# kawshik8/GAN-Image-Captioning

Measured on NVIDIA B200. Metric: adversarial_train_steps_per_sec, higher is better.
Workload: dtype bf16 operands on the discriminator's highway/dx/dW_h contractions, tf32 on the others (fp32 accumulate)

## Files before the change

gan-image-captioning_b200/_lib.py:

```python
from __future__ import annotations

import ctypes as C
import os
import re

HERE = os.path.dirname(os.path.abspath(__file__))
LIB_PATH = os.path.join(HERE, "libgic_b200.so")
HEADER = os.path.join(os.path.dirname(HERE), "include", "gic_b200.h")

GEMM_FP32, GEMM_TF32, GEMM_BF16 = 0, 1, 3
LOSS_TYPES = {"standard": 0, "JS": 1, "KL": 2, "hinge": 3, "tv": 4, "rsgan": 5}

_lib = None


class AttnBlock(C.Structure):
    _fields_ = [("grid", C.c_void_p), ("P", C.c_int), ("Cf", C.c_int), ("Da", C.c_int), ("W_k", C.c_void_p),
                ("W_v", C.c_void_p), ("W_q", C.c_void_p), ("w_e", C.c_void_p), ("saved", C.c_void_p), ("ws", C.c_void_p),
                ("dW_k", C.c_void_p), ("dW_v", C.c_void_p), ("dW_q", C.c_void_p), ("dw_e", C.c_void_p)]


def attn_block(grid, W_k, W_v, W_q, w_e, saved, ws=None, dW_k=None, dW_v=None, dW_q=None, dw_e=None):
    B, Pn, Cf = grid.shape
    return AttnBlock(ptr(grid), Pn, Cf, W_k.shape[0], ptr(W_k), ptr(W_v), ptr(W_q), ptr(w_e), ptr(saved), ptr(ws),
# ... 47 lines not shown
    L.gic_encoder_bwd.argtypes = [I, P, P, P, P, P, P, P, I, I, I, P, P, P, P, P, I, P]
    L.gic_encoder_bn_running_update.argtypes = [P, P, I, F, F, F, P, P, P, P]
    L.gic_encoder_fwd_eval.argtypes = [I, P, I, I, I, P, P, P, P, F, P, P, P, P, P]
    L.gic_sample_step.argtypes = [I, P, P, F, I, I, I, I, P, P, P, P, I, P, P]
    for f in (L.gic_decode_saved_floats, L.gic_decode_fwd_workspace_floats, L.gic_decode_bwd_workspace_floats,
              L.gic_disc_saved_floats, L.gic_disc_fwd_workspace_floats, L.gic_disc_bwd_workspace_floats,
              L.gic_disc_bwd_demb_offset_floats):
        f.restype = Z
    L.gic_decode_saved_floats.argtypes = [I] * 5
    L.gic_decode_fwd_workspace_floats.argtypes = [I] * 3
    L.gic_decode_bwd_workspace_floats.argtypes = [I] * 6
    L.gic_disc_saved_floats.argtypes = [I] * 5
    L.gic_disc_fwd_workspace_floats.argtypes = [I]
    L.gic_disc_bwd_workspace_floats.argtypes = [I] * 5
    L.gic_disc_bwd_demb_offset_floats.argtypes = [I] * 5
    L.gic_decode_sample_bwd_factored.argtypes = [I, P, P, P, I, P, P, P, P, P, P, F, I, I, I, I, I, I, P, P, P, P, P, P,
                                                 P, P, P, P, I, P]
    L.gic_decode_sample_fwd.argtypes = [I, P, P, P, P, P, P, P, P, P, F, I, P, I, I, I, I, I, I, P, P, P, P, P]
    L.gic_decode_sample_bwd.argtypes = [I, P, P, P, P, P, P, P, F, I, I, I, I, I, I, I, P, P, P, P, P, P, P, P, P, P,
                                        I, P]
    L.gic_disc_fwd.argtypes = [I, P, P, I, I, I, I, I, I, P, P, P, P, P, P, P, P, P, I, P, P, I, P, F, P, P, P, P]
    L.gic_disc_bwd.argtypes = [I, P, P, F, P, P, I, I, I, I, I, I, P, P, P, P, P, P, P, P, I, P, P, P, P, P, P, P, P,
                               P, P, P, P, P, P, I, I, P]
    L.gic_gan_loss_fwd_bwd.argtypes = [I, P, P, P, I, P, P, P, P, P]
    L.gic_grad_sqnorm.argtypes = [P, Z, P, P]
    L.gic_clip_adam.argtypes = [P, P, P, P, Z, P, F, F, I, F, F, F, F, P]
    L.gic_clip_adam_dyn.argtypes = [P, P, P, P, Z, P, F, F, P, F, F, F, P]
    L.gic_decode_sample_cdf_fwd.argtypes = [I, P, P, P, P, P, P, P, P, P, P, I, I, I, I, I, I, P, P, P, P, P, P]
    L.gic_attn_saved_floats.restype = Z
    L.gic_attn_saved_floats.argtypes = [I] * 5
    L.gic_attn_bwd_workspace_floats.restype = Z
    L.gic_attn_bwd_workspace_floats.argtypes = [I] * 5
    L.gic_decode_sample_fwd_attn.argtypes = [P] + [I, P, P, P, P, P, P, P, P, P, F, I, P, I, I, I, I, I, I, P, P, P, P, P]
    L.gic_decode_sample_bwd_attn.argtypes = [P, I, P, P, P, P, I, P, P, P, P, P, P, F, I, I, I, I, I, I, I, P, P, P, P, P,
                                             P, P, P, P, P, P]
    L.gic_sample_cdf_step.argtypes = [P, P, I, I, I, I, P, P, P, P, P, I, P, P]
    L.gic_decode_rollouts_workspace_floats.restype = Z
    L.gic_decode_rollouts_workspace_floats.argtypes = [I] * 6
    L.gic_decode_rollouts.argtypes = [I, P, P, P, P, P, P, P, P, P, P, I, I, I, I, I, I, P, P, P]
    L.gic_rollout_rewards.argtypes = [P, P, I, I, I, I, P, P]
    L.gic_ce_loss_fwd_bwd.argtypes = [P, P, I, I, I, P, P, P]
    L.gic_pg_loss_fwd_bwd.argtypes = [P, P, P, I, I, I, I, P, P, P, P]
    L.gic_set_temperature_device.restype = None
    L.gic_set_temperature_device.argtypes = [P]
    L.gic_disc_prepared_floats.restype = Z
    L.gic_disc_prepared_floats.argtypes = [I]
# ... 199 lines not shown
```

gan-image-captioning_b200/csrc/capi.cu:

```cuda
#include "../../include/gic_b200.h"
#include <stdlib.h>
#include <new>

#include "gic_internal.cuh"

namespace gic {
int gather_rows(const float*, const int64_t*, int, int, int, float*, cudaStream_t);
int vec_add(const float*, const float*, int, float*, cudaStream_t);
int sample_step(bool, const float*, const float*, float, int, int, int, int, float*, int64_t*, const int64_t*,
                const float*, int, float*, cudaStream_t, bool fast_math = false);
int softmax_bwd(const float*, const float*, float, int, int, float*, cudaStream_t);
int rowdot(const float*, const float*, int, int, float*, cudaStream_t);
int sample_cdf_step(const float*, const float*, int, int, int, int, long long, float*, int64_t*, float*, const int64_t*,
                    const float*, int, float*, cudaStream_t);
int rollout_init(const float*, const float*, const int64_t*, const float*, int, int, int, int, int, int, int, float*,
                 float*, float*, int64_t*, cudaStream_t);
int softmax_bwd_dot(const float*, const float*, const float*, float, int, int, float*, cudaStream_t);
int softmax_bwd_dot_bf16(const float*, const float*, const float*, float, int, int, void*, int, cudaStream_t);
int colsum_bf16(const void*, int, int, int, bool, float*, cudaStream_t);
int embed_scatter(const float*, const int64_t*, int, int, int, int, float*, float*, cudaStream_t);
int bn_fwd(const float*, int, int, const float*, const float*, float, float*, float*, float*, cudaStream_t);
int bn_bwd(const float*, const float*, int, int, const float*, const float*, const float*, float*, float*, float*,
           cudaStream_t);
int lstm_cell_fwd(const float*, const float*, int, int, float*, float*, float*, float*, int, int, cudaStream_t);
// ... 52 lines not shown
int pack_captions(const int32_t*, const int32_t*, int, int, int64_t*, int32_t*, cudaStream_t);
const float* temperature_device();
void disc_set_prepared(const float*);
int disc_prepare(int, const float*, const float*, const float*, int, const float*, const float*, int, float*, cudaStream_t);
size_t disc_fwd_workspace_floats(int);
const char* last_error();
unsigned long long launch_count();
unsigned long long kernel_launches(const char*);
int kernel_names(char*, int);
void prof_begin();
void prof_end(double*, double*, unsigned long long*);
int disc_fwd_entry(int mode, const float* inp_soft, const int64_t* ids, int N, int L, int V, int De, int R,
                   int n_groups, const int* fs, const int* nf, const float* W_e, const float* const* cw,
                   const float* const* cb, const float* W_h, const float* b_h, const float* W_f, const float* b_f,
                   int Hd, const float* W_o, const float* b_o, int n_heads, const uint8_t* const* keep, float drop_p,
                   float* const* logits, float* saved, float* ws, cudaStream_t s);
int disc_bwd_entry(int mode, const float* dlogits, const uint8_t* keep, float drop_p, const float* inp_soft,
                   const int64_t* ids, int N, int L, int V, int De, int R, int n_groups, const int* fs, const int* nf,
                   const float* W_e, const float* const* cw, const float* const* cb, const float* W_h,
                   const float* W_f, const float* b_f, int Hd, const float* W_o, const float* b_o, const float* saved,
                   float* ws, float* dW_e, float* const* dcw, float* const* dcb, float* dW_h, float* db_h,
                   float* dW_f, float* db_f, float* dW_o, float* db_o, float* dinp, int want_param, int accumulate,
                   cudaStream_t s);

static size_t a4(size_t x) { return (x + 3) & ~(size_t)3; }

struct AttnLayout {
  size_t Ak, Av, q, alpha, total;
  size_t dAk, dAv, dq, ds, ws_total;
  AttnLayout(int B, int L, int P, int Da, int E) {
    Ak = 0; Av = a4((size_t)B * P * Da); q = Av + a4((size_t)B * P * E); alpha = q + a4((size_t)L * B * Da);
    total = alpha + a4((size_t)L * B * P);
    dAk = 0; dAv = a4((size_t)B * P * Da); dq = dAv + a4((size_t)B * P * E); ds = dq + a4((size_t)L * B * Da);
    ws_total = ds + a4((size_t)L * B * P);
  }
};

struct DecodeSaved {
  size_t xs, hs0, cs0, acts0, per_layer, htop, total;
  DecodeSaved(int B, int L, int E, int H, int layers) {
    const size_t BH = (size_t)B * H;
    xs = 0;
    size_t off = a4((size_t)L * B * E);
    hs0 = off;
    cs0 = hs0 + a4((size_t)(L + 1) * BH);
    acts0 = cs0 + a4((size_t)(L + 1) * BH);
// ... 703 lines not shown
                 int n_groups, const int* filter_sizes, const int* num_filters, const float* W_e,
                 const float* const* conv_w, const float* const* conv_b, const float* W_h, const float* b_h,
                 const float* W_f, const float* b_f, int Hd, const float* W_o, const float* b_o, int n_heads,
                 const uint8_t* const* keep, float drop_p, float* const* logits, float* saved, float* workspace,
                 gic_stream_t stream) {
  GIC_TRY(require_device());
  return disc_fwd_entry(mode, inp_soft, ids, N, L, V, De, R, n_groups, filter_sizes, num_filters, W_e, conv_w, conv_b,
                        W_h, b_h, W_f, b_f, Hd, W_o, b_o, n_heads, keep, drop_p, logits, saved, workspace, S(stream));
}

int gic_disc_bwd(int mode, const float* dlogits, const uint8_t* keep, float drop_p, const float* inp_soft,
                 const int64_t* ids, int N, int L, int V, int De, int R, int n_groups, const int* filter_sizes,
                 const int* num_filters, const float* W_e, const float* const* conv_w, const float* const* conv_b,
                 const float* W_h, const float* W_f, const float* b_f, int Hd, const float* W_o, const float* b_o,
                 const float* saved, float* workspace, float* dW_e, float* const* dconv_w, float* const* dconv_b,
                 float* dW_h, float* db_h, float* dW_f, float* db_f, float* dW_o, float* db_o, float* dinp,
                 int want_param, int accumulate, gic_stream_t stream) {
  GIC_TRY(require_device());
  return disc_bwd_entry(mode, dlogits, keep, drop_p, inp_soft, ids, N, L, V, De, R, n_groups, filter_sizes,
                        num_filters, W_e, conv_w, conv_b, W_h, W_f, b_f, Hd, W_o, b_o, saved, workspace, dW_e, dconv_w,
                        dconv_b, dW_h, db_h, dW_f, db_f, dW_o, db_o, dinp, want_param, accumulate, S(stream));
}

int gic_gan_loss_fwd_bwd(int loss_type, const float* d_out_real, const float* d_out_fake, const float* g_out, int n,
                         float* losses, float* dd_real, float* dd_fake, float* dg_out, gic_stream_t stream) {
  GIC_TRY(require_device());
  return gan_loss(loss_type, d_out_real, d_out_fake, g_out, n, losses, dd_real, dd_fake, dg_out, S(stream));
}

int gic_grad_sqnorm(const float* g, size_t n, float* sqnorm, gic_stream_t stream) {
  GIC_TRY(require_device());
  return grad_sqnorm(g, n, sqnorm, S(stream));
}

int gic_clip_adam(float* p, const float* g, float* m, float* v, size_t n, const float* sqnorm, float max_norm,
                  float grad_scale, int step, float lr, float beta1, float beta2, float eps, gic_stream_t stream) {
  GIC_TRY(require_device());
  return clip_adam(p, g, m, v, n, sqnorm, max_norm, grad_scale, step, lr, beta1, beta2, eps, nullptr, S(stream));
}

int gic_clip_adam_dyn(float* p, const float* g, float* m, float* v, size_t n, const float* sqnorm, float max_norm,
                      float grad_scale, const float* bias_corr_dev, float beta1, float beta2, float eps,
                      gic_stream_t stream) {
  GIC_TRY(require_device());
  GIC_REQUIRE(bias_corr_dev, GIC_ERR_NULL, "clip_adam_dyn: NULL bias_corr_dev");
  return clip_adam(p, g, m, v, n, sqnorm, max_norm, grad_scale, 0, 0.f, beta1, beta2, eps, bias_corr_dev, S(stream));
// ... 59 lines not shown
```

gan-image-captioning_b200/csrc/disc.cu:

```cuda
#include <stdlib.h>

#include "gic_internal.cuh"

namespace gic {

constexpr int MAX_GROUPS = 8;

__device__ __forceinline__ unsigned long long pack2(float lo, float hi) {
  unsigned long long r;
  asm("mov.b64 %0, {%1, %2};" : "=l"(r) : "f"(lo), "f"(hi));
  return r;
}
__device__ __forceinline__ void unpack2(unsigned long long v, float& lo, float& hi) {
  asm("mov.b64 {%0, %1}, %2;" : "=f"(lo), "=f"(hi) : "l"(v));
}
__device__ __forceinline__ unsigned long long ffma2(unsigned long long a, unsigned long long b, unsigned long long c) {
  unsigned long long d;
  asm("fma.rn.f32x2 %0, %1, %2, %3;" : "=l"(d) : "l"(a), "l"(b), "l"(c));
  return d;
}

__device__ __forceinline__ unsigned short f2bf(float x) {
  unsigned int u = __float_as_uint(x);
  u += 0x7fffu + ((u >> 16) & 1u);
// ... 462 lines not shown
      const int row = rb + j;
      const bool ok = active && row < r1;
      const size_t i = (size_t)row * F + c;
      gv[j] = ok ? dx[i] + dx2[i] : 0.f;
      av[j] = ok ? (int)arg[i] : ARG_DEAD;
    }
    __syncthreads();
#pragma unroll
    for (int j = 0; j < DW_RC; ++j) {
      if (av[j] != ARG_DEAD && gv[j] != 0.f) {
        const float* e0 = sm + j * LE + av[j] * es;
#pragma unroll
        for (int k = 0; k < BWD_KMAX; ++k)
          if (k < fk) dw[k] = fmaf(gv[j], e0[k], dw[k]);
        dbias += gv[j];
      }
    }
  }
  if (!active) return;
#pragma unroll
  for (int k = 0; k < BWD_KMAX; ++k)
    if (k < fk) atomicAdd(g.dw[gi] + cin * fk + k, dw[k]);
  atomicAdd(g.db[gi] + cin, dbias);
}

__global__ void __launch_bounds__(256)
head_collapse_kernel(const float* __restrict__ W_f, const float* __restrict__ b_f,
                     const float* __restrict__ w_o, const float* __restrict__ b_o, int F,
                     int Hd, float* __restrict__ weff ) {
  __shared__ float part[8][33];
  const int lane = threadIdx.x & 31, w = threadIdx.x >> 5;
  const int j = blockIdx.x * 32 + lane;
  float s = 0.f;
  if (j < F) {
#pragma unroll 4
    for (int k = w; k < Hd; k += 8) s = fmaf(w_o[k], W_f[(size_t)k * F + j], s);
  } else if (j == F) {
    for (int k = w; k < Hd; k += 8) s = fmaf(w_o[k], b_f[k], s);
  }
  part[w][lane] = s;
  __syncthreads();
  if (w == 0 && j <= F) {
    float t = (j == F) ? b_o[0] : 0.f;
#pragma unroll
    for (int i = 0; i < 8; ++i) t += part[i][lane];
    weff[j] = t;
// ... 256 lines not shown
static size_t align4(size_t x) { return (x + 3) & ~(size_t)3; }

static inline int bf_pitch(int F) { return ((F + 63) / 64) * 64; }

size_t disc_saved_floats(int N, int L, int De, int R, int F) {
  const size_t rows = (size_t)N * R;
  return align4((size_t)N * L * De) + 2 * align4(rows * F) + align4((rows * F + 3) / 4) + align4(rows * bf_pitch(F) / 2);
}
size_t disc_fwd_workspace_floats(int F) { return align4((size_t)F + 1) + align4((size_t)F * bf_pitch(F) / 2); }
size_t disc_bwd_workspace_floats(int N, int L, int De, int R, int F) {
  const size_t rows = (size_t)N * R;
  const size_t dh = align4(rows * F) > align4(rows * bf_pitch(F) / 2) ? align4(rows * F) : align4(rows * bf_pitch(F) / 2);
  return align4((size_t)F + 1) + dh + align4(rows * F) + 2 * align4(F) + align4((size_t)N * L * De) +
         align4((size_t)F * bf_pitch(F) / 2) + align4(rows * F);
}

int disc_fill_groups(ConvGroups& g, int ngroups, const int* fs, const int* nf, const float* const* cw,
                     const float* const* cb, float* const* dcw, float* const* dcb, int es) {
  GIC_REQUIRE(ngroups >= 1 && ngroups <= MAX_GROUPS, GIC_ERR_SHAPE, "disc: 1..%d filter groups supported", MAX_GROUPS);
  g.ngroups = ngroups; g.F = 0; g.kmax = 0;
  for (int i = 0; i < MAX_GROUPS; ++i) { g.w[i] = g.b[i] = nullptr; g.dw[i] = g.db[i] = nullptr; g.f[i] = g.n[i] = g.col0[i] = 0; }
  for (int i = 0; i < ngroups; ++i) {
    GIC_REQUIRE(fs[i] >= 1 && nf[i] >= 1, GIC_ERR_SHAPE, "disc: bad filter group %d", i);
    GIC_REQUIRE(cw[i] && cb[i], GIC_ERR_NULL, "disc: NULL conv weights for group %d", i);
    g.w[i] = cw[i]; g.b[i] = cb[i];
    g.dw[i] = dcw ? dcw[i] : nullptr; g.db[i] = dcb ? dcb[i] : nullptr;
    g.f[i] = fs[i]; g.n[i] = nf[i]; g.col0[i] = g.F; g.F += nf[i];
    if (fs[i] * es > g.kmax) g.kmax = fs[i] * es;
  }
  return GIC_OK;
}

void disc_set_prepared(const float* prep) { ctx().prepared = prep; }
#define g_prepared (ctx().prepared)

int disc_prepare(int mode, const float* W_h, const float* W_f, const float* b_f, int Hd, const float* W_o,
                 const float* b_o, int F, float* prep, cudaStream_t s) {
  GIC_REQUIRE(W_h && W_f && b_f && W_o && b_o && prep, GIC_ERR_NULL, "disc_prepare: NULL pointer");
  GIC_REQUIRE(F >= 1 && Hd >= 1, GIC_ERR_SHAPE, "disc_prepare: bad shape");
  head_collapse_kernel<<<cdiv(F + 1, 32), 256, 0, s>>>(W_f, b_f, W_o, b_o, F, Hd, prep);
  GIC_TRY(check_launch("head_collapse_kernel"));
  if (mode == GEMM_BF16 && (F % 4 == 0)) {
    unsigned short* W_h_bf = reinterpret_cast<unsigned short*>(prep + align4((size_t)F + 1));
    GIC_TRY(f32_to_bf16(W_h, F, F, F, W_h_bf, bf_pitch(F), s));
  }
  return GIC_OK;
}

// ... 78 lines not shown
  }
  HeadPtrs hp;
  hp.n = n_heads;
  for (int m = 0; m < MAX_HEADS; ++m) {
    hp.keep[m] = (m < n_heads && keep) ? keep[m] : nullptr;
    hp.logits[m] = (m < n_heads) ? logits[m] : nullptr;
  }
  ProfScope prof(PROF_HEAD, (8.0 + n_heads) * rows * d.F, s);
  bool vec = (d.F % 4 == 0) && d.F <= 4 * 32 * 8;
  for (int m = 0; m < n_heads; ++m) vec = vec && (!hp.keep[m] || (reinterpret_cast<uintptr_t>(hp.keep[m]) & 3u) == 0);
  if (vec) {
    const int nq = cdiv(d.F / 4, 32);
    const int grid = cdiv((long long)rows, 8);
    const float dsc = 1.f / (1.f - drop_p);
    const bool fast = (mode == GEMM_TF32 || mode == GEMM_BF16);
#define GIC_HF(NQ_) do { if (fast) head_fwd_vec_kernel<NQ_, true><<<grid, 256, 0, s>>>(hpre, pooled, (int)rows, d.F, weff, dsc, hp); \
                         else head_fwd_vec_kernel<NQ_, false><<<grid, 256, 0, s>>>(hpre, pooled, (int)rows, d.F, weff, dsc, hp); } while (0)
    if (nq <= 2) GIC_HF(2); else if (nq <= 4) GIC_HF(4); else GIC_HF(8);
#undef GIC_HF
  } else {
    head_fwd_kernel<<<cdiv((long long)rows, 8), 256, 0, s>>>(hpre, pooled, (int)rows, d.F, weff, 1.f / (1.f - drop_p), hp);
  }
  return check_launch("head_fwd_kernel");
}

int disc_backward(int mode, const float* dlogit, const uint8_t* keep, float drop_p, const float* inp_soft,
                  const int64_t* ids, const DiscDims& d, ConvGroups& g, const float* W_e, const float* W_h,
                  const float* W_f, const float* b_f, const float* W_o, const float* b_o, const float* saved,
                  float* ws, float* dW_e, float* dW_h, float* db_h, float* dW_f, float* db_f, float* dW_o,
                  float* db_o, float* dinp, int want_param, int accumulate, cudaStream_t s) {
  const size_t rows = d.rows();
  if (d.N == 0) return GIC_OK;
  const float* emb = saved;
  const float* pooled = emb + align4((size_t)d.N * d.L * d.De);
  const float* hpre = pooled + align4(rows * d.F);
  const uint8_t* arg = reinterpret_cast<const uint8_t*>(hpre + align4(rows * d.F));
  const bool bf = (mode == GEMM_BF16) && (d.F % 4 == 0) && (!keep || (reinterpret_cast<uintptr_t>(keep) & 3u) == 0);
  const int Fp = bf_pitch(d.F);
  const unsigned short* pooled_bf =
      reinterpret_cast<const unsigned short*>(reinterpret_cast<const float*>(arg) + align4((rows * d.F + 3) / 4));
  const float* prep = g_prepared;
  const float* weff = prep ? prep : ws;
  float* dh = ws + align4((size_t)d.F + 1);
  const size_t dh_floats = align4(rows * d.F) > align4(rows * Fp / 2) ? align4(rows * d.F) : align4(rows * Fp / 2);
  float* dx = dh + dh_floats;
  float* sacc = dx + align4(rows * d.F);
// ... 28 lines not shown
    const int colb = cdiv(d.F, 256);
    int chunks = max(1, (4 * num_sms()) / colb);
    int rpc = cdiv((long long)rows, chunks);
    chunks = cdiv((long long)rows, rpc);
    head_bwd_kernel<<<dim3(colb, chunks), 256, 0, s>>>(dlogit, keep, 1.f / (1.f - drop_p), hpre, pooled, (int)rows,
                                                      d.F, weff, rpc, dh, dx, sacc, dbh);
    GIC_TRY(check_launch("head_bwd_kernel"));
  }
  if (want_param) {
    head_param_grads_kernel<<<d.Hd, 256, 0, s>>>(dlogit, (int)rows, sacc, dbh, W_f, b_f, W_o, d.F, d.Hd, beta, dW_f,
                                                db_f, dW_o, db_o, db_h);
    GIC_TRY(check_launch("head_param_grads_kernel"));
    if (bf)
      GIC_TRY(gemm_bf16(true, false, d.F, d.F, (int)rows, 1.f, dh, Fp, pooled_bf, Fp, beta, dW_h, d.F, nullptr, s, PROF_GEMM_D));
    else
      GIC_TRY(gemm(mode, true, false, d.F, d.F, (int)rows, 1.f, dh, d.F, pooled, d.F, beta, dW_h, d.F, nullptr, s, PROF_GEMM_D));
  }
  if (bf) {
    if (!prep) GIC_TRY(f32_to_bf16(W_h, d.F, d.F, d.F, W_h_bf_ws, Fp, s));
    GIC_TRY(gemm_bf16(false, false, (int)rows, d.F, d.F, 1.f, dh, Fp, W_h_bf, Fp, 0.f, dxg, d.F, nullptr, s, PROF_GEMM_D));
  } else {
    GIC_TRY(gemm(mode, false, false, (int)rows, d.F, d.F, 1.f, dh, d.F, W_h, d.F, 0.f, dxg, d.F, nullptr, s, PROF_GEMM_D));
  }
  {
    GIC_REQUIRE(g.kmax <= BWD_KMAX, GIC_ERR_SHAPE, "disc bwd: filter_size*emb_dim_single <= %d supported", BWD_KMAX);
    if (want_param && !accumulate) {
      for (int i = 0; i < g.ngroups; ++i) {
        cudaMemsetAsync(g.dw[i], 0, (size_t)g.n[i] * g.f[i] * d.es * sizeof(float), s);
        cudaMemsetAsync(g.db[i], 0, (size_t)g.n[i] * sizeof(float), s);
      }
    }
    {
      const size_t fixed = ((size_t)g.kmax + 1) * d.F * 4;
      const size_t per_warp = (size_t)d.L * d.es * 32 * 4;
      int nwarps = 8;
      while (nwarps > 1 && fixed + nwarps * per_warp > 100 * 1024) nwarps >>= 1;
      const size_t smem = fixed + nwarps * per_warp;
      GIC_REQUIRE(smem <= 200 * 1024, GIC_ERR_SHAPE, "disc bwd: L*emb_dim_single too large for shared memory");
      const int grid = min(cdiv((long long)rows, nwarps), 4 * num_sms());
      bool vec = (d.F % 4 == 0) && aligned16(dx) && aligned16(dxg) && ((reinterpret_cast<uintptr_t>(arg) & 3u) == 0);
      for (int i = 0; i < g.ngroups; ++i) vec = vec && (g.n[i] % 4 == 0);
      static bool attr = false;
      if (!attr) {
        cudaFuncSetAttribute(conv_pool_bwd_demb_kernel<true, true>, cudaFuncAttributeMaxDynamicSharedMemorySize, 200 * 1024);
        cudaFuncSetAttribute(conv_pool_bwd_demb_kernel<true, false>, cudaFuncAttributeMaxDynamicSharedMemorySize, 200 * 1024);
        cudaFuncSetAttribute(conv_pool_bwd_demb_kernel<false, true>, cudaFuncAttributeMaxDynamicSharedMemorySize, 200 * 1024);
        cudaFuncSetAttribute(conv_pool_bwd_demb_kernel<false, false>, cudaFuncAttributeMaxDynamicSharedMemorySize, 200 * 1024);
        attr = true;
      }
#define GIC_DEMB(ES1_, VEC_) conv_pool_bwd_demb_kernel<ES1_, VEC_><<<grid, nwarps * 32, smem, s>>>(arg, dx, dxg, (int)rows, d.L, d.De, d.R, d.es, g, demb)
      if (d.es == 1) { if (vec) GIC_DEMB(true, true); else GIC_DEMB(true, false); }
      else { if (vec) GIC_DEMB(false, true); else GIC_DEMB(false, false); }
#undef GIC_DEMB
      GIC_TRY(check_launch("conv_pool_bwd_demb_kernel"));
    }
    if (want_param) {
      const int colb = cdiv(d.F, 256);
      int per_sm = 4;
      { const int o = option("GIC_DW_CTAS_PER_SM", 0); if (o > 0) per_sm = o; }
      int chunks = max(1, (per_sm * num_sms()) / colb);
      int rpc = cdiv((long long)rows, chunks);
      rpc = ((rpc + DW_RC - 1) / DW_RC) * DW_RC;
      chunks = cdiv((long long)rows, rpc);
      const size_t smem = (size_t)DW_RC * d.L * d.es * 4;
      GIC_REQUIRE(smem <= 48 * 1024, GIC_ERR_SHAPE, "disc bwd: L*emb_dim_single too large for shared memory");
      if (d.es == 1)
        conv_pool_bwd_dw_kernel<true><<<dim3(colb, chunks), 256, smem, s>>>(emb, arg, dx, dxg, (int)rows, d.L, d.De, d.R, d.es, g, rpc);
      else
        conv_pool_bwd_dw_kernel<false><<<dim3(colb, chunks), 256, smem, s>>>(emb, arg, dx, dxg, (int)rows, d.L, d.De, d.R, d.es, g, rpc);
      GIC_TRY(check_launch("conv_pool_bwd_dw_kernel"));
    }
  }
  if (want_param) {
    if (inp_soft) {
      GIC_TRY(gemm(mode, true, false, d.De, d.V, d.N * d.L, 1.f, demb, d.De, inp_soft, d.V, beta, dW_e, d.V, nullptr, s));
    } else {
      if (!accumulate) cudaMemsetAsync(dW_e, 0, (size_t)d.De * d.V * sizeof(float), s);
      const int tot = d.N * d.L * d.De;
      disc_embed_ids_bwd_kernel<<<cdiv(tot, 256), 256, 0, s>>>(ids, d.N * d.L, d.V, d.De, demb, dW_e);
      GIC_TRY(check_launch("disc_embed_ids_bwd_kernel"));
    }
  }
  if (dinp) {
    GIC_TRY(gemm(mode, false, false, d.N * d.L, d.V, d.De, 1.f, demb, d.De, W_e, d.V, 0.f, dinp, d.V, nullptr, s));
  }
  return GIC_OK;
}

static int disc_dims(DiscDims& d, int N, int L, int V, int De, int R, int Hd, const ConvGroups& g) {
  GIC_REQUIRE(N >= 0 && L >= 1 && V >= 1 && De >= 1 && R >= 1 && Hd >= 1, GIC_ERR_SHAPE, "disc: bad shape");
  GIC_REQUIRE(De % R == 0, GIC_ERR_SHAPE, "disc: disc_embed_dim %d not divisible by disc_num_rep %d", De, R);
  d.N = N; d.L = L; d.V = V; d.De = De; d.R = R; d.es = De / R; d.F = g.F; d.Hd = Hd; d.ngroups = g.ngroups;
  d.kmax = g.kmax;
  for (int i = 0; i < g.ngroups; ++i)
    GIC_REQUIRE(L >= g.f[i], GIC_ERR_SHAPE, "disc: caption length %d shorter than filter size %d", L, g.f[i]);
// ... 23 lines not shown

int disc_bwd_entry(int mode, const float* dlogits, const uint8_t* keep, float drop_p, const float* inp_soft,
                   const int64_t* ids, int N, int L, int V, int De, int R, int n_groups, const int* fs, const int* nf,
                   const float* W_e, const float* const* cw, const float* const* cb, const float* W_h,
                   const float* W_f, const float* b_f, int Hd, const float* W_o, const float* b_o, const float* saved,
                   float* ws, float* dW_e, float* const* dcw, float* const* dcb, float* dW_h, float* db_h,
                   float* dW_f, float* db_f, float* dW_o, float* db_o, float* dinp, int want_param, int accumulate,
                   cudaStream_t s) {
  GIC_REQUIRE((inp_soft != nullptr) != (ids != nullptr), GIC_ERR_NULL, "disc_bwd: exactly one of inp_soft / ids");
  GIC_REQUIRE(dlogits && fs && nf && cw && cb && W_e && W_h && W_f && b_f && W_o && b_o && saved && ws, GIC_ERR_NULL,
              "disc_bwd: NULL pointer");
  GIC_REQUIRE(!want_param || (dW_e && dcw && dcb && dW_h && db_h && dW_f && db_f && dW_o && db_o), GIC_ERR_NULL,
              "disc_bwd: NULL gradient buffer");
  GIC_REQUIRE(!(dinp && ids), GIC_ERR_UNSUPPORTED, "disc_bwd: hard-token input has no gradient");
  const int es = (R > 0 && De % R == 0) ? De / R : 1;
  ConvGroups g;
  GIC_TRY(disc_fill_groups(g, n_groups, fs, nf, cw, cb, want_param ? dcw : nullptr, want_param ? dcb : nullptr, es));
  DiscDims d;
  GIC_TRY(disc_dims(d, N, L, V, De, R, Hd, g));
  return disc_backward(mode, dlogits, keep, drop_p, inp_soft, ids, d, g, W_e, W_h, W_f, b_f, W_o, b_o, saved, ws, dW_e,
                       dW_h, db_h, dW_f, db_f, dW_o, db_o, dinp, want_param, accumulate, s);
}

}
```

include/gic_b200.h:

```cpp
#ifndef GIC_B200_H_
#define GIC_B200_H_

#include <stddef.h>
#include <stdint.h>

#ifdef __cplusplus
extern "C" {
#endif

typedef void* gic_stream_t;

#define GIC_OK 0
#define GIC_ERR_SHAPE 1
#define GIC_ERR_NULL 2
#define GIC_ERR_CUDA 3
#define GIC_ERR_WORKSPACE 4
#define GIC_ERR_ARCH 5
#define GIC_ERR_UNSUPPORTED 6

#define GIC_GEMM_FP32 0
#define GIC_GEMM_TF32 1
#define GIC_GEMM_BF16 3

#define GIC_LOSS_STANDARD 0
// ... 64 lines not shown
                                   float temperature, int B, int L, int V, int E, int H, int layers, const float* saved,
                                   float* workspace, float* dW_emb, float* const* dW_ih, float* const* dW_hh,
                                   float* const* db_ih, float* const* db_hh, float* dW_out, float* db_out,
                                   float* dfeatures, int accumulate, gic_stream_t stream);

size_t gic_disc_saved_floats(int N, int L, int De, int R, int F);
size_t gic_disc_fwd_workspace_floats(int F);
int gic_disc_fwd(int mode, const float* inp_soft, const int64_t* ids, int N, int L, int V, int De, int R,
                 int n_groups, const int* filter_sizes, const int* num_filters, const float* W_e ,
                 const float* const* conv_w, const float* const* conv_b, const float* W_h ,
                 const float* b_h, const float* W_f , const float* b_f, int Hd, const float* W_o ,
                 const float* b_o, int n_heads, const uint8_t* const* keep, float drop_p, float* const* logits,
                 float* saved, float* workspace, gic_stream_t stream);

size_t gic_disc_bwd_workspace_floats(int N, int L, int De, int R, int F);
size_t gic_disc_bwd_demb_offset_floats(int N, int L, int De, int R, int F);
int gic_disc_bwd(int mode, const float* dlogits, const uint8_t* keep, float drop_p, const float* inp_soft,
                 const int64_t* ids, int N, int L, int V, int De, int R, int n_groups, const int* filter_sizes,
                 const int* num_filters, const float* W_e, const float* const* conv_w, const float* const* conv_b,
                 const float* W_h, const float* W_f, const float* b_f, int Hd, const float* W_o, const float* b_o,
                 const float* saved, float* workspace, float* dW_e, float* const* dconv_w, float* const* dconv_b,
                 float* dW_h, float* db_h, float* dW_f, float* db_f, float* dW_o, float* db_o, float* dinp,
                 int want_param, int accumulate, gic_stream_t stream);

int gic_gan_loss_fwd_bwd(int loss_type, const float* d_out_real, const float* d_out_fake, const float* g_out, int n,
                         float* losses, float* dd_real, float* dd_fake, float* dg_out, gic_stream_t stream);

int gic_grad_sqnorm(const float* g, size_t n, float* sqnorm, gic_stream_t stream);
int gic_clip_adam(float* p, const float* g, float* m, float* v, size_t n, const float* sqnorm, float max_norm,
                  float grad_scale, int step, float lr, float beta1, float beta2, float eps, gic_stream_t stream);

int gic_ce_loss_fwd_bwd(const float* logits , const int64_t* targets , int B, int L, int V,
                        float* loss , float* dlogits , gic_stream_t stream);

int gic_sample_cdf_step(const float* logits, const float* u, int B, int V, int L, int t, float* out, int64_t* ids,
                        float* logp, const int64_t* forced_ids, const float* embed, int E, float* x_next,
                        gic_stream_t stream);
int gic_decode_sample_cdf_fwd(int mode, const float* features, const float* W_emb, const float* const* W_ih,
                              const float* const* W_hh, const float* const* b_ih, const float* const* b_hh,
                              const float* W_out, const float* b_out, const float* u, const int64_t* forced_ids, int B,
                              int L, int V, int E, int H, int layers, float* logits_out, int64_t* ids, float* logp,
                              float* saved, float* workspace, gic_stream_t stream);
size_t gic_decode_rollouts_workspace_floats(int B, int L, int V, int E, int H, int n_roll);
int gic_decode_rollouts(int mode, const float* saved, const int64_t* main_ids, const float* W_emb, const float* W_ih,
                        const float* W_hh, const float* b_ih, const float* b_hh, const float* W_out,
                        const float* b_out, const float* u_roll, int B, int L, int V, int E, int H, int n_roll,
// ... 110 lines not shown
```

Measured before the change: 459.3.

## Fuse conv-pool backward demb and weight-gradient passes into one kernel

```diff
diff --git a/gan-image-captioning_b200/_lib.py b/gan-image-captioning_b200/_lib.py
--- a/gan-image-captioning_b200/_lib.py
+++ b/gan-image-captioning_b200/_lib.py
@@ -93,6 +93,7 @@
     L.gic_disc_fwd.argtypes = [I, P, P, I, I, I, I, I, I, P, P, P, P, P, P, P, P, P, I, P, P, I, P, F, P, P, P, P]
     L.gic_disc_bwd.argtypes = [I, P, P, F, P, P, I, I, I, I, I, I, P, P, P, P, P, P, P, P, I, P, P, P, P, P, P, P, P,
                                P, P, P, P, P, P, I, I, P]
+    L.gic_conv_pool_bwd.argtypes = [P, P, P, P, I, I, I, I, I, P, P, P, P, P, P, I, I, P]
     L.gic_gan_loss_fwd_bwd.argtypes = [I, P, P, P, I, P, P, P, P, P]
     L.gic_grad_sqnorm.argtypes = [P, Z, P, P]
     L.gic_clip_adam.argtypes = [P, P, P, P, Z, P, F, F, I, F, F, F, F, P]
diff --git a/gan-image-captioning_b200/csrc/capi.cu b/gan-image-captioning_b200/csrc/capi.cu
--- a/gan-image-captioning_b200/csrc/capi.cu
+++ b/gan-image-captioning_b200/csrc/capi.cu
@@ -98,6 +98,9 @@
                    float* ws, float* dW_e, float* const* dcw, float* const* dcb, float* dW_h, float* db_h,
                    float* dW_f, float* db_f, float* dW_o, float* db_o, float* dinp, int want_param, int accumulate,
                    cudaStream_t s);
+int conv_pool_bwd_entry(const uint8_t* arg, const float* dx, const float* dx2, const float* emb, int N, int L, int De, int R,
+                        int n_groups, const int* fs, const int* nf, const float* const* cw, float* const* dcw,
+                        float* const* dcb, float* demb, int want_param, int accumulate, cudaStream_t s);
 
 static size_t a4(size_t x) { return (x + 3) & ~(size_t)3; }
 
@@ -847,6 +850,15 @@
                         dconv_b, dW_h, db_h, dW_f, db_f, dW_o, db_o, dinp, want_param, accumulate, S(stream));
 }
 
+int gic_conv_pool_bwd(const uint8_t* arg, const float* dx, const float* dx2, const float* emb, int N, int L, int De, int R,
+                      int n_groups, const int* filter_sizes, const int* num_filters, const float* const* conv_w,
+                      float* const* dconv_w, float* const* dconv_b, float* demb, int want_param, int accumulate,
+                      gic_stream_t stream) {
+  GIC_TRY(require_device());
+  return conv_pool_bwd_entry(arg, dx, dx2, emb, N, L, De, R, n_groups, filter_sizes, num_filters, conv_w, dconv_w, dconv_b,
+                             demb, want_param, accumulate, S(stream));
+}
+
 int gic_gan_loss_fwd_bwd(int loss_type, const float* d_out_real, const float* d_out_fake, const float* g_out, int n,
                          float* losses, float* dd_real, float* dd_fake, float* dg_out, gic_stream_t stream) {
   GIC_TRY(require_device());
diff --git a/gan-image-captioning_b200/csrc/disc.cu b/gan-image-captioning_b200/csrc/disc.cu
--- a/gan-image-captioning_b200/csrc/disc.cu
+++ b/gan-image-captioning_b200/csrc/disc.cu
@@ -508,6 +508,164 @@
   for (int k = 0; k < BWD_KMAX; ++k)
     if (k < fk) atomicAdd(g.dw[gi] + cin * fk + k, dw[k]);
   atomicAdd(g.db[gi] + cin, dbias);
+}
+
+template <bool WANT_PARAM, int QPL, int KM>
+__global__ void __launch_bounds__(256, QPL * (KM + 1) <= 12 ? 2 : 1)
+conv_pool_bwd_fused_kernel(const float* __restrict__ emb, const uint8_t* __restrict__ arg, const float* __restrict__ dx,
+                           const float* __restrict__ dx2, int rows, int L, int R, ConvGroups g, int qs,
+                           int rows_per_cta, float* __restrict__ demb, int demb_atomic) {
+  extern __shared__ __align__(16) float sm[];
+  const int F = g.F, F4 = F >> 2;
+  const int nwarps = blockDim.x >> 5, warp = threadIdx.x >> 5, lane = threadIdx.x & 31;
+  const int q_lo = blockIdx.x * qs, nq = min(qs, F4 - q_lo);
+  float4* wk_s = reinterpret_cast<float4*>(sm);
+  float4* red_s = wk_s + (size_t)KM * qs;
+  float* priv = reinterpret_cast<float*>(red_s + (WANT_PARAM ? (size_t)(KM + 1) * qs : 0)) + (size_t)warp * 33 * 32;
+  float* erow = priv + 32 * 32;
+  for (int i = threadIdx.x; i < KM * nq; i += blockDim.x) {
+    const int k = i / nq, ql = i % nq, c = 4 * (q_lo + ql);
+    int gi = 0;
+    while (gi + 1 < g.ngroups && c >= g.col0[gi + 1]) ++gi;
+    const int f = g.f[gi];
+    const float* w = g.w[gi] + (size_t)(c - g.col0[gi]) * f + k;
+    wk_s[k * qs + ql] = (k < f) ? make_float4(w[0], w[f], w[2 * f], w[3 * f]) : make_float4(0.f, 0.f, 0.f, 0.f);
+  }
+  if (WANT_PARAM)
+    for (int i = threadIdx.x; i < (KM + 1) * qs; i += blockDim.x) red_s[i] = make_float4(0.f, 0.f, 0.f, 0.f);
+  int fk[QPL];
+#pragma unroll
+  for (int j = 0; j < QPL; ++j) {
+    const int ql = 32 * j + lane;
+    fk[j] = 0;
+    if (ql < nq) {
+      const int c = 4 * (q_lo + ql);
+      int gi = 0;
+      while (gi + 1 < g.ngroups && c >= g.col0[gi + 1]) ++gi;
+      fk[j] = g.f[gi];
+    }
+  }
+  float4 dw[QPL][KM + 1];
+  if (WANT_PARAM) {
+#pragma unroll
+    for (int j = 0; j < QPL; ++j)
+#pragma unroll
+      for (int k = 0; k <= KM; ++k) dw[j][k] = make_float4(0.f, 0.f, 0.f, 0.f);
+  }
+  __syncthreads();
+
+  const int r0 = blockIdx.y * rows_per_cta, r1 = min(rows, r0 + rows_per_cta);
+  float4 gv[QPL], hv[QPL];
+  uint32_t av[QPL];
+  float ev = 0.f;
+  auto load = [&](int row) {
+    const size_t base = (size_t)row * F;
+    const float4* dx4 = reinterpret_cast<const float4*>(dx + base) + q_lo;
+    const float4* dy4 = reinterpret_cast<const float4*>(dx2 + base) + q_lo;
+    const uint32_t* a4 = reinterpret_cast<const uint32_t*>(arg + base) + q_lo;
+    const bool live = row < r1;
+#pragma unroll
+    for (int j = 0; j < QPL; ++j) {
+      const int ql = 32 * j + lane;
+      const bool ok = live && ql < nq;
+      gv[j] = ok ? dx4[ql] : make_float4(0.f, 0.f, 0.f, 0.f);
+      hv[j] = ok ? dy4[ql] : make_float4(0.f, 0.f, 0.f, 0.f);
+      av[j] = ok ? __ldg(a4 + ql) : 0xffffffffu;
+    }
+    if (WANT_PARAM) ev = (live && lane < L) ? emb[((size_t)(row / R) * L + lane) * R + row % R] : 0.f;
+  };
+  int row = r0 + warp;
+  load(row);
+  for (; row < r1; row += nwarps) {
+    float4 gc[QPL];
+    uint32_t ac[QPL];
+#pragma unroll
+    for (int j = 0; j < QPL; ++j) {
+      gc[j] = make_float4(gv[j].x + hv[j].x, gv[j].y + hv[j].y, gv[j].z + hv[j].z, gv[j].w + hv[j].w);
+      ac[j] = av[j];
+    }
+    if (WANT_PARAM) erow[lane] = ev;
+    load(row + nwarps);
+    for (int t = 0; t < L; ++t) priv[t * 32 + lane] = 0.f;
+    __syncwarp();
+#pragma unroll
+    for (int j = 0; j < QPL; ++j) {
+      const float gg[4] = {gc[j].x, gc[j].y, gc[j].z, gc[j].w};
+      const int aa[4] = {(int)(ac[j] & 0xffu), (int)((ac[j] >> 8) & 0xffu), (int)((ac[j] >> 16) & 0xffu), (int)(ac[j] >> 24)};
+      bool on[4];
+      bool any = false;
+#pragma unroll
+      for (int e = 0; e < 4; ++e) { on[e] = (aa[e] != ARG_DEAD) && (gg[e] != 0.f); any |= on[e]; }
+      if (!any) continue;
+      const int f = fk[j];
+      float4 w4[KM];
+#pragma unroll
+      for (int k = 0; k < KM; ++k) if (k < f) w4[k] = wk_s[k * qs + 32 * j + lane];
+#pragma unroll
+      for (int e = 0; e < 4; ++e) {
+        if (!on[e]) continue;
+        float* p = priv + aa[e] * 32 + lane;
+        const float* er = erow + aa[e];
+#pragma unroll
+        for (int k = 0; k < KM; ++k) {
+          if (k < f) {
+            const float wk = e == 0 ? w4[k].x : e == 1 ? w4[k].y : e == 2 ? w4[k].z : w4[k].w;
+            p[k * 32] = fmaf(wk, gg[e], p[k * 32]);
+            if (WANT_PARAM) {
+              float& d = e == 0 ? dw[j][k].x : e == 1 ? dw[j][k].y : e == 2 ? dw[j][k].z : dw[j][k].w;
+              d = fmaf(gg[e], er[k], d);
+            }
+          }
+        }
+        if (WANT_PARAM) {
+          float& d = e == 0 ? dw[j][KM].x : e == 1 ? dw[j][KM].y : e == 2 ? dw[j][KM].z : dw[j][KM].w;
+          d += gg[e];
+        }
+      }
+    }
+    __syncwarp();
+    if (lane < L) {
+      float acc = 0.f;
+#pragma unroll 8
+      for (int i = 0; i < 32; ++i) acc += priv[lane * 32 + ((i + lane) & 31)];
+      float* o = demb + ((size_t)(row / R) * L + lane) * R + row % R;
+      if (!demb_atomic) *o = acc;
+      else if (acc != 0.f) atomicAdd(o, acc);
+    }
+    __syncwarp();
+  }
+  if (!WANT_PARAM) return;
+  for (int w = 0; w < nwarps; ++w) {
+    if (warp == w) {
+#pragma unroll
+      for (int j = 0; j < QPL; ++j) {
+        const int ql = 32 * j + lane;
+        if (ql >= nq) continue;
+#pragma unroll
+        for (int k = 0; k <= KM; ++k) {
+          float4 v = red_s[k * qs + ql];
+          v.x += dw[j][k].x; v.y += dw[j][k].y; v.z += dw[j][k].z; v.w += dw[j][k].w;
+          red_s[k * qs + ql] = v;
+        }
+      }
+    }
+    __syncthreads();
+  }
+  for (int i = threadIdx.x; i < (KM + 1) * nq; i += blockDim.x) {
+    const int k = i / nq, ql = i % nq, c = 4 * (q_lo + ql);
+    int gi = 0;
+    while (gi + 1 < g.ngroups && c >= g.col0[gi + 1]) ++gi;
+    const int f = g.f[gi], cin = c - g.col0[gi];
+    const float4 v = red_s[k * qs + ql];
+    const float vv[4] = {v.x, v.y, v.z, v.w};
+    if (k == KM) {
+#pragma unroll
+      for (int e = 0; e < 4; ++e) atomicAdd(g.db[gi] + cin + e, vv[e]);
+    } else if (k < f) {
+#pragma unroll
+      for (int e = 0; e < 4; ++e) atomicAdd(g.dw[gi] + (size_t)(cin + e) * f + k, vv[e]);
+    }
+  }
 }
 
 __global__ void __launch_bounds__(256)
@@ -810,8 +968,8 @@
   for (int i = 0; i < MAX_GROUPS; ++i) { g.w[i] = g.b[i] = nullptr; g.dw[i] = g.db[i] = nullptr; g.f[i] = g.n[i] = g.col0[i] = 0; }
   for (int i = 0; i < ngroups; ++i) {
     GIC_REQUIRE(fs[i] >= 1 && nf[i] >= 1, GIC_ERR_SHAPE, "disc: bad filter group %d", i);
-    GIC_REQUIRE(cw[i] && cb[i], GIC_ERR_NULL, "disc: NULL conv weights for group %d", i);
-    g.w[i] = cw[i]; g.b[i] = cb[i];
+    GIC_REQUIRE(cw[i] && (!cb || cb[i]), GIC_ERR_NULL, "disc: NULL conv weights for group %d", i);
+    g.w[i] = cw[i]; g.b[i] = cb ? cb[i] : nullptr;
     g.dw[i] = dcw ? dcw[i] : nullptr; g.db[i] = dcb ? dcb[i] : nullptr;
     g.f[i] = fs[i]; g.n[i] = nf[i]; g.col0[i] = g.F; g.F += nf[i];
     if (fs[i] * es > g.kmax) g.kmax = fs[i] * es;
@@ -936,6 +1094,100 @@
     head_fwd_kernel<<<cdiv((long long)rows, 8), 256, 0, s>>>(hpre, pooled, (int)rows, d.F, weff, 1.f / (1.f - drop_p), hp);
   }
   return check_launch("head_fwd_kernel");
+}
+
+int conv_pool_bwd(const uint8_t* arg, const float* dx, const float* dx2, const float* emb, int N, int L, int De, int R,
+                  const ConvGroups& g, float* demb, int want_param, int accumulate, cudaStream_t s) {
+  const int es = De / R;
+  const size_t rows = (size_t)N * R;
+  GIC_REQUIRE(g.kmax <= BWD_KMAX, GIC_ERR_SHAPE, "disc bwd: filter_size*emb_dim_single <= %d supported", BWD_KMAX);
+  if (want_param && !accumulate) {
+    for (int i = 0; i < g.ngroups; ++i) {
+      cudaMemsetAsync(g.dw[i], 0, (size_t)g.n[i] * g.f[i] * es * sizeof(float), s);
+      cudaMemsetAsync(g.db[i], 0, (size_t)g.n[i] * sizeof(float), s);
+    }
+  }
+  if (rows == 0) return GIC_OK;
+  bool vec = (g.F % 4 == 0) && aligned16(dx) && aligned16(dx2) && ((reinterpret_cast<uintptr_t>(arg) & 3u) == 0);
+  for (int i = 0; i < g.ngroups; ++i) vec = vec && (g.n[i] % 4 == 0);
+  if (vec && es == 1 && L <= 32 && option("GIC_CONV_BWD_FUSED", 1) != 0) {
+    const int km = g.kmax <= 5 ? 5 : 8;
+    int qpl = km == 5 ? 4 : 2;
+    if (km == 5 && option("GIC_CONV_BWD_QPL", 0) == 2) qpl = 2;
+    const int F4 = g.F / 4;
+    const int slices = cdiv(F4, 32 * qpl), qs = cdiv(F4, slices);
+    const size_t smem = (size_t)km * qs * 16 + (want_param ? (size_t)(km + 1) * qs * 16 : 0) + (size_t)8 * 33 * 32 * 4;
+    static bool attr = false;
+    if (!attr) {
+#define GIC_FATTR(P_, Q_, K_) cudaFuncSetAttribute(conv_pool_bwd_fused_kernel<P_, Q_, K_>, cudaFuncAttributeMaxDynamicSharedMemorySize, 200 * 1024)
+      GIC_FATTR(true, 4, 5); GIC_FATTR(true, 2, 5); GIC_FATTR(true, 2, 8);
+      GIC_FATTR(false, 4, 5); GIC_FATTR(false, 2, 5); GIC_FATTR(false, 2, 8);
+#undef GIC_FATTR
+      attr = true;
+    }
+#define GIC_FUSED(P_, Q_, K_)                                                                                               \
+    do {                                                                                                                    \
+      static size_t occ_smem = 0;                                                                                           \
+      static int occ = 1;                                                                                                   \
+      if (occ_smem != smem) {                                                                                               \
+        cudaOccupancyMaxActiveBlocksPerMultiprocessor(&occ, conv_pool_bwd_fused_kernel<P_, Q_, K_>, 256, smem);           \
+        occ = max(occ, 1);                                                                                                  \
+        occ_smem = smem;                                                                                                    \
+      }                                                                                                                     \
+      int chunks = max(1, (occ * num_sms()) / slices);                                                                      \
+      const int rpc = (int)cdiv((long long)rows, chunks);                                                                   \
+      chunks = (int)cdiv((long long)rows, rpc);                                                                             \
+      conv_pool_bwd_fused_kernel<P_, Q_, K_><<<dim3(slices, chunks), 256, smem, s>>>(emb, arg, dx, dx2, (int)rows, L, R,   \
+                                                                                      g, qs, rpc, demb, slices > 1);       \
+    } while (0)
+    if (slices > 1) cudaMemsetAsync(demb, 0, (size_t)N * L * De * sizeof(float), s);
+    if (want_param) {
+      if (km == 8) GIC_FUSED(true, 2, 8); else if (qpl == 2) GIC_FUSED(true, 2, 5); else GIC_FUSED(true, 4, 5);
+    } else {
+      if (km == 8) GIC_FUSED(false, 2, 8); else if (qpl == 2) GIC_FUSED(false, 2, 5); else GIC_FUSED(false, 4, 5);
+    }
+#undef GIC_FUSED
+    return check_launch("conv_pool_bwd_fused_kernel");
+  }
+  {
+    const size_t fixed = ((size_t)g.kmax + 1) * g.F * 4;
+    const size_t per_warp = (size_t)L * es * 32 * 4;
+    int nwarps = 8;
+    while (nwarps > 1 && fixed + nwarps * per_warp > 100 * 1024) nwarps >>= 1;
+    const size_t smem = fixed + nwarps * per_warp;
+    GIC_REQUIRE(smem <= 200 * 1024, GIC_ERR_SHAPE, "disc bwd: L*emb_dim_single too large for shared memory");
+    const int grid = min(cdiv((long long)rows, nwarps), 4 * num_sms());
+    static bool attr = false;
+    if (!attr) {
+      cudaFuncSetAttribute(conv_pool_bwd_demb_kernel<true, true>, cudaFuncAttributeMaxDynamicSharedMemorySize, 200 * 1024);
+      cudaFuncSetAttribute(conv_pool_bwd_demb_kernel<true, false>, cudaFuncAttributeMaxDynamicSharedMemorySize, 200 * 1024);
+      cudaFuncSetAttribute(conv_pool_bwd_demb_kernel<false, true>, cudaFuncAttributeMaxDynamicSharedMemorySize, 200 * 1024);
+      cudaFuncSetAttribute(conv_pool_bwd_demb_kernel<false, false>, cudaFuncAttributeMaxDynamicSharedMemorySize, 200 * 1024);
+      attr = true;
+    }
+#define GIC_DEMB(ES1_, VEC_) conv_pool_bwd_demb_kernel<ES1_, VEC_><<<grid, nwarps * 32, smem, s>>>(arg, dx, dx2, (int)rows, L, De, R, es, g, demb)
+    if (es == 1) { if (vec) GIC_DEMB(true, true); else GIC_DEMB(true, false); }
+    else { if (vec) GIC_DEMB(false, true); else GIC_DEMB(false, false); }
+#undef GIC_DEMB
+    GIC_TRY(check_launch("conv_pool_bwd_demb_kernel"));
+  }
+  if (want_param) {
+    const int colb = cdiv(g.F, 256);
+    int per_sm = 4;
+    { const int o = option("GIC_DW_CTAS_PER_SM", 0); if (o > 0) per_sm = o; }
+    int chunks = max(1, (per_sm * num_sms()) / colb);
+    int rpc = cdiv((long long)rows, chunks);
+    rpc = ((rpc + DW_RC - 1) / DW_RC) * DW_RC;
+    chunks = cdiv((long long)rows, rpc);
+    const size_t smem = (size_t)DW_RC * L * es * 4;
+    GIC_REQUIRE(smem <= 48 * 1024, GIC_ERR_SHAPE, "disc bwd: L*emb_dim_single too large for shared memory");
+    if (es == 1)
+      conv_pool_bwd_dw_kernel<true><<<dim3(colb, chunks), 256, smem, s>>>(emb, arg, dx, dx2, (int)rows, L, De, R, es, g, rpc);
+    else
+      conv_pool_bwd_dw_kernel<false><<<dim3(colb, chunks), 256, smem, s>>>(emb, arg, dx, dx2, (int)rows, L, De, R, es, g, rpc);
+    GIC_TRY(check_launch("conv_pool_bwd_dw_kernel"));
+  }
+  return GIC_OK;
 }
 
 int disc_backward(int mode, const float* dlogit, const uint8_t* keep, float drop_p, const float* inp_soft,
@@ -1010,55 +1262,7 @@
   } else {
     GIC_TRY(gemm(mode, false, false, (int)rows, d.F, d.F, 1.f, dh, d.F, W_h, d.F, 0.f, dxg, d.F, nullptr, s, PROF_GEMM_D));
   }
-  {
-    GIC_REQUIRE(g.kmax <= BWD_KMAX, GIC_ERR_SHAPE, "disc bwd: filter_size*emb_dim_single <= %d supported", BWD_KMAX);
-    if (want_param && !accumulate) {
-      for (int i = 0; i < g.ngroups; ++i) {
-        cudaMemsetAsync(g.dw[i], 0, (size_t)g.n[i] * g.f[i] * d.es * sizeof(float), s);
-        cudaMemsetAsync(g.db[i], 0, (size_t)g.n[i] * sizeof(float), s);
-      }
-    }
-    {
-      const size_t fixed = ((size_t)g.kmax + 1) * d.F * 4;
-      const size_t per_warp = (size_t)d.L * d.es * 32 * 4;
-      int nwarps = 8;
-      while (nwarps > 1 && fixed + nwarps * per_warp > 100 * 1024) nwarps >>= 1;
-      const size_t smem = fixed + nwarps * per_warp;
-      GIC_REQUIRE(smem <= 200 * 1024, GIC_ERR_SHAPE, "disc bwd: L*emb_dim_single too large for shared memory");
-      const int grid = min(cdiv((long long)rows, nwarps), 4 * num_sms());
-      bool vec = (d.F % 4 == 0) && aligned16(dx) && aligned16(dxg) && ((reinterpret_cast<uintptr_t>(arg) & 3u) == 0);
-      for (int i = 0; i < g.ngroups; ++i) vec = vec && (g.n[i] % 4 == 0);
-      static bool attr = false;
-      if (!attr) {
-        cudaFuncSetAttribute(conv_pool_bwd_demb_kernel<true, true>, cudaFuncAttributeMaxDynamicSharedMemorySize, 200 * 1024);
-        cudaFuncSetAttribute(conv_pool_bwd_demb_kernel<true, false>, cudaFuncAttributeMaxDynamicSharedMemorySize, 200 * 1024);
-        cudaFuncSetAttribute(conv_pool_bwd_demb_kernel<false, true>, cudaFuncAttributeMaxDynamicSharedMemorySize, 200 * 1024);
-        cudaFuncSetAttribute(conv_pool_bwd_demb_kernel<false, false>, cudaFuncAttributeMaxDynamicSharedMemorySize, 200 * 1024);
-        attr = true;
-      }
-#define GIC_DEMB(ES1_, VEC_) conv_pool_bwd_demb_kernel<ES1_, VEC_><<<grid, nwarps * 32, smem, s>>>(arg, dx, dxg, (int)rows, d.L, d.De, d.R, d.es, g, demb)
-      if (d.es == 1) { if (vec) GIC_DEMB(true, true); else GIC_DEMB(true, false); }
-      else { if (vec) GIC_DEMB(false, true); else GIC_DEMB(false, false); }
-#undef GIC_DEMB
-      GIC_TRY(check_launch("conv_pool_bwd_demb_kernel"));
-    }
-    if (want_param) {
-      const int colb = cdiv(d.F, 256);
-      int per_sm = 4;
-      { const int o = option("GIC_DW_CTAS_PER_SM", 0); if (o > 0) per_sm = o; }
-      int chunks = max(1, (per_sm * num_sms()) / colb);
-      int rpc = cdiv((long long)rows, chunks);
-      rpc = ((rpc + DW_RC - 1) / DW_RC) * DW_RC;
-      chunks = cdiv((long long)rows, rpc);
-      const size_t smem = (size_t)DW_RC * d.L * d.es * 4;
-      GIC_REQUIRE(smem <= 48 * 1024, GIC_ERR_SHAPE, "disc bwd: L*emb_dim_single too large for shared memory");
-      if (d.es == 1)
-        conv_pool_bwd_dw_kernel<true><<<dim3(colb, chunks), 256, smem, s>>>(emb, arg, dx, dxg, (int)rows, d.L, d.De, d.R, d.es, g, rpc);
-      else
-        conv_pool_bwd_dw_kernel<false><<<dim3(colb, chunks), 256, smem, s>>>(emb, arg, dx, dxg, (int)rows, d.L, d.De, d.R, d.es, g, rpc);
-      GIC_TRY(check_launch("conv_pool_bwd_dw_kernel"));
-    }
-  }
+  GIC_TRY(conv_pool_bwd(arg, dx, dxg, emb, d.N, d.L, d.De, d.R, g, demb, want_param, accumulate, s));
   if (want_param) {
     if (inp_soft) {
       GIC_TRY(gemm(mode, true, false, d.De, d.V, d.N * d.L, 1.f, demb, d.De, inp_soft, d.V, beta, dW_e, d.V, nullptr, s));
@@ -1128,4 +1332,20 @@
                        dW_h, db_h, dW_f, db_f, dW_o, db_o, dinp, want_param, accumulate, s);
 }
 
-}
+int conv_pool_bwd_entry(const uint8_t* arg, const float* dx, const float* dx2, const float* emb, int N, int L, int De, int R,
+                        int n_groups, const int* fs, const int* nf, const float* const* cw, float* const* dcw,
+                        float* const* dcb, float* demb, int want_param, int accumulate, cudaStream_t s) {
+  GIC_REQUIRE(arg && dx && dx2 && emb && fs && nf && cw && demb, GIC_ERR_NULL, "conv_pool_bwd: NULL pointer");
+  GIC_REQUIRE(!want_param || (dcw && dcb), GIC_ERR_NULL, "conv_pool_bwd: NULL gradient buffer");
+  GIC_REQUIRE(N >= 0 && L >= 1 && R >= 1 && De >= 1 && De % R == 0, GIC_ERR_SHAPE, "conv_pool_bwd: bad shape");
+  GIC_REQUIRE(L <= 254, GIC_ERR_SHAPE, "conv_pool_bwd: caption length <= 254 supported");
+  ConvGroups g;
+  GIC_TRY(disc_fill_groups(g, n_groups, fs, nf, cw, nullptr, want_param ? dcw : nullptr, want_param ? dcb : nullptr, De / R));
+  for (int i = 0; i < n_groups; ++i) {
+    GIC_REQUIRE(L >= fs[i], GIC_ERR_SHAPE, "conv_pool_bwd: caption length %d shorter than filter size %d", L, fs[i]);
+    GIC_REQUIRE(!want_param || (dcw[i] && dcb[i]), GIC_ERR_NULL, "conv_pool_bwd: NULL gradient of group %d", i);
+  }
+  return conv_pool_bwd(arg, dx, dx2, emb, N, L, De, R, g, demb, want_param, accumulate, s);
+}
+
+}
diff --git a/include/gic_b200.h b/include/gic_b200.h
--- a/include/gic_b200.h
+++ b/include/gic_b200.h
@@ -110,6 +110,11 @@
                  const float* saved, float* workspace, float* dW_e, float* const* dconv_w, float* const* dconv_b,
                  float* dW_h, float* db_h, float* dW_f, float* db_f, float* dW_o, float* db_o, float* dinp,
                  int want_param, int accumulate, gic_stream_t stream);
+
+int gic_conv_pool_bwd(const uint8_t* arg, const float* dx, const float* dx2, const float* emb, int N, int L, int De, int R,
+                      int n_groups, const int* filter_sizes, const int* num_filters, const float* const* conv_w,
+                      float* const* dconv_w, float* const* dconv_b, float* demb, int want_param, int accumulate,
+                      gic_stream_t stream);
 
 int gic_gan_loss_fwd_bwd(int loss_type, const float* d_out_real, const float* d_out_fake, const float* g_out, int n,
                          float* losses, float* dd_real, float* dd_fake, float* dg_out, gic_stream_t stream);
diff --git a/profiles/conv_bwd_bench.py b/profiles/conv_bwd_bench.py
--- /dev/null
+++ b/profiles/conv_bwd_bench.py
@@ -0,0 +1,118 @@
+import argparse
+import json
+import os
+import statistics
+import subprocess
+import sys
+import tempfile
+
+import torch
+
+ROOT = os.path.dirname(os.path.dirname(os.path.abspath(__file__)))
+sys.path.insert(0, ROOT)
+import gic_b200
+from gic_b200 import _lib
+from gic_b200.discriminator import disc_fwd_raw
+
+HBM_PEAK = 7.7e12
+COPY_RATE = 6.5e12
+CALLS, ROUNDS = 50, 7
+SHAPES = {"c2": (256, 20), "c5": (4096, 32)}
+FSZ, NFL, R, V = [3, 4, 5], [300, 300, 300], 64, 10000
+
+
+def a4(x):
+    return (x + 3) & ~3
+
+
+def setup(N, L, dev):
+    g = torch.Generator(device=dev).manual_seed(0)
+    De, Fd, Hd = R, sum(NFL), 100
+    u = lambda *s: (torch.rand(*s, generator=g, device=dev) - 0.5) * 0.1
+    W_e = u(De, V) * 10
+    cw = [u(n, 1, f, 1).contiguous() for n, f in zip(NFL, FSZ)]
+    cb = [u(n) for n in NFL]
+    W_h, b_h, W_f, b_f, W_o, b_o = u(Fd, Fd), u(Fd), u(Hd, Fd), u(Hd), u(1, Hd), u(1)
+    ids = torch.randint(0, V, (N, L), generator=g, device=dev)
+    lib = _lib.lib()
+    _, saved = disc_fwd_raw(lib, gic_b200.GEMM_BF16, None, ids, N, L, V, De, R, FSZ, NFL, W_e, cw, cb, W_h, b_h, W_f, b_f,
+                            W_o, b_o, [None], 0.0, dev)
+    rows = N * R
+    emb = saved[:N * L * De].view(N, L, De)
+    off = a4(N * L * De) + 2 * a4(rows * Fd)
+    arg = saved[off:off + a4((rows * Fd + 3) // 4)].view(torch.uint8)[:rows * Fd].view(rows, Fd)
+    dx = torch.randn(rows, Fd, generator=g, device=dev)
+    dx2 = torch.randn(rows, Fd, generator=g, device=dev)
+    live = float(((arg != 255) & ((dx + dx2) != 0)).float().mean())
+    dW = [torch.zeros(n, f, device=dev) for n, f in zip(NFL, FSZ)]
+    db = [torch.zeros(n, device=dev) for n in NFL]
+    demb = torch.empty(N, L, De, device=dev)
+    return dict(N=N, L=L, De=De, rows=rows, F=Fd, arg=arg, dx=dx, dx2=dx2, emb=emb, cw=cw, dW=dW, db=db, demb=demb,
+                live=live, keep=saved)
+
+
+def call(t, want_param):
+    lib = _lib.lib()
+    _lib.check(lib.gic_conv_pool_bwd(_lib.ptr(t["arg"]), _lib.ptr(t["dx"]), _lib.ptr(t["dx2"]), _lib.ptr(t["emb"]), t["N"],
+                                     t["L"], t["De"], R, len(FSZ), _lib.int_array(FSZ), _lib.int_array(NFL),
+                                     _lib.ptr_array(t["cw"]), _lib.ptr_array(t["dW"]), _lib.ptr_array(t["db"]),
+                                     _lib.ptr(t["demb"]), want_param, 1, _lib.stream()), "gic_conv_pool_bwd")
+
+
+VARIANTS = {"fused": dict(GIC_CONV_BWD_FUSED=1), "fused_qpl2": dict(GIC_CONV_BWD_FUSED=1, GIC_CONV_BWD_QPL=2),
+            "pair": dict(GIC_CONV_BWD_FUSED=0)}
+
+
+def time_round(t, want_param, opts):
+    with _lib.options(**opts):
+        call(t, want_param)
+        torch.cuda.synchronize()
+        e0, e1 = torch.cuda.Event(enable_timing=True), torch.cuda.Event(enable_timing=True)
+        e0.record()
+        for _ in range(CALLS):
+            call(t, want_param)
+        e1.record()
+        torch.cuda.synchronize()
+    return e0.elapsed_time(e1) * 1e3 / CALLS
+
+
+def main():
+    ap = argparse.ArgumentParser()
+    ap.add_argument("--out", default=os.environ.get("GIC_REPORT_DIR", tempfile.gettempdir()))
+    args = ap.parse_args()
+    _lib.require_cuda()
+    dev = torch.device("cuda:0")
+    smi = subprocess.run(["nvidia-smi", "--query-gpu=name,power.limit,clocks.max.sm", "--format=csv,noheader"],
+                         capture_output=True, text=True).stdout.strip()
+    rep = dict(gpu=smi, calls=CALLS, rounds=ROUNDS, hbm_peak_Bps=HBM_PEAK, copy_rate_Bps=COPY_RATE, results=[])
+    print("gpu:", smi)
+    for name, (N, L) in SHAPES.items():
+        t = setup(N, L, dev)
+        rows, F = t["rows"], t["F"]
+        stream_bytes = rows * F * 9
+        small = 2 * N * L * R * 4
+        print("%s: N %d L %d rows %d F %d live fraction %.4f" % (name, N, L, rows, F, t["live"]))
+        for want_param in (1, 0):
+            times = {v: [] for v in VARIANTS}
+            for _ in range(ROUNDS):
+                for v, opts in VARIANTS.items():
+                    times[v].append(time_round(t, want_param, opts))
+            for v in VARIANTS:
+                us = statistics.median(times[v])
+                passes = 2 if (v == "pair" and want_param) else 1
+                nbytes = passes * stream_bytes + small
+                floor_us = stream_bytes / HBM_PEAK * 1e6
+                r = dict(shape=name, N=N, L=L, want_param=want_param, variant=v, us=us, us_all=times[v], bytes=nbytes,
+                         GBps=nbytes / us * 1e-3, frac_hbm_peak=floor_us / us, live_fraction=t["live"])
+                rep["results"].append(r)
+                print("  want_param=%d %-10s %8.1f us  %7.1f GB/s  one-pass HBM floor %.1f us (%.0f %% of it)" % (
+                    want_param, v, us, r["GBps"], floor_us, 100 * r["frac_hbm_peak"]))
+        del t
+        torch.cuda.empty_cache()
+    os.makedirs(args.out, exist_ok=True)
+    with open(os.path.join(args.out, "conv_bwd_bench.json"), "w") as f:
+        json.dump(rep, f, indent=1)
+
+
+if __name__ == "__main__":
+    main()
```

Result: no change. 457.5 (median of 6 runs) (-0.4%).
